# SerCharles/CN-RMA

Hardware: AMD Instinct MI355X
Metric: scenes/sec fwd (40-view->192^3 voxel): dense unprojection + RMA + voxelise + FCAF3D + decode (higher is better)
Workload: dtype f32 (sparse conv f16x3: 22-bit operands, fp32 accumulate; value_f32_conv = exact fp32); 1 GPU; NS: 40 views x 256 ch x 480x640 fp32 maps (channels_last) -> grid 192x192x192, N=300, max_points=500000, FCAF3D MinkResNet34 + head, 1 HIP graph per scene, 3 in flight; M_rows=72216505, M_selected=500000, M_unique=496819

## Files before the change

### cn-rma_amd/csrc/sparse.hip

```cpp
#include <cstdio>
#include <type_traits>
#include "common.h"

#include <hipcub/hipcub.hpp>

namespace {

struct UniqueWs {
  int32_t* slot;
  int32_t* idx;
  uint8_t* flag;
  void* scan;
  uint64_t* key_a; uint64_t* key_b;
  int32_t* val_a; int32_t* val_b;
  void* sort_tmp; size_t sort_tmp_bytes;
  int32_t* range_err;
};

size_t sort_temp_bytes(int64_t n) {
  size_t bytes = 0;
  hipError_t e = hipcub::DeviceRadixSort::SortPairs(nullptr, bytes, (const uint64_t*)nullptr, (uint64_t*)nullptr,
                                                    (const int32_t*)nullptr, (int32_t*)nullptr, (int)n, 0, 64, nullptr);
  if (e != hipSuccess || bytes == 0) bytes = (size_t)n * 16 + (1u << 20);
  (void)hipGetLastError();
// ... 1140 lines not shown
#pragma unroll
      for (int j = 0; j < 4; ++j) {
        float x = v[j];
        if (p.scale) x = x * scv[j];
        if (p.shift) x = x + shv[j];
        if (p.residual) x = x + rsv[j];
        v[j] = apply_act(x, p.act);
        mx = fmaxf(mx, fabsf(v[j]));
        if (p.out_split) store_split(p.out_split, t / p.Cout, p.Cout, col + j, v[j]);
      }
      *reinterpret_cast<float4*>(p.out + t) = make_float4(v[0], v[1], v[2], v[3]);
    } else {
      for (int j = 0; j < 4 && t + j < total; ++j) {
        float x = 0.0f;
        for (int z = 0; z < p.splits; ++z) x += p.slab[(int64_t)z * slab_stride + t + j];
        const int col = (int)((t + j) % p.Cout);
        if (p.scale) x = x * p.scale[col];
        if (p.shift) x = x + p.shift[col];
        if (p.residual) x = x + p.residual[t + j];
        x = apply_act(x, p.act);
        mx = fmaxf(mx, fabsf(x));
        p.out[t + j] = x;
      }
    }
  }
  if (p.out_amax != nullptr) {
    __shared__ float sh4[4];
    block_amax_publish(p.out_amax, mx, sh4);
  }
}

int choose_splits(int64_t rows, int Cout, int K, int bm, int bn, size_t ws_bytes) {
  if (K <= 1) return 1;
  const int64_t tiles = ceil_div(rows, bm) * ceil_div(Cout, bn);
  if (tiles >= 384) return 1;
  int s = (int)ceil_div(768, tiles);
  if (s > K) s = K;
  const size_t per = (size_t)rows * Cout * sizeof(float);
  if (per == 0) return 1;
  const int64_t fit = (int64_t)(ws_bytes / per);
  if (s > fit) s = (int)fit;
  return s < 2 ? 1 : s;
}

#ifdef CNRMA_EXPERIMENTS
#include "sparse_exp_ws.inc"
#endif

constexpr int CONV_XCD_ORDER = 0;
#ifdef CNRMA_EXPERIMENTS
constexpr int CONV_WS_SLOTS = 0;
#endif

struct ConvTune { int shape = -1; int splits = -1; int pf = -1; int ablate = 0; int ws = -1; int xcd = -1; int go = -1; int nb = -1; };
#ifdef CNRMA_EXPERIMENTS
static ConvTune g_conv_tune;
#define CNRMA_CONV_TUNE g_conv_tune
#else
static constexpr ConvTune k_conv_tune{};
#define CNRMA_CONV_TUNE k_conv_tune
#endif

enum ConvMode { CONV_EXACT = 0, CONV_F16X3 = 1, CONV_BF16 = 2 };

static int64_t capped_blocks(int64_t threads, int64_t cap) {
  const int64_t b = ceil_div(threads, 256);
  return b > cap ? cap : b;
}

static ConvArgs conv_args(const float* in, int Cin, const int32_t* nbr, int K, int Cout, float* out, int64_t no_cap,
                          const int32_t* no_dev, void* slab = nullptr) {
  ConvArgs p;
  p.in = in; p.Cin = Cin; p.nbr = nbr; p.K = K; p.Cout = Cout; p.out = out; p.no_cap = no_cap; p.no_dev = no_dev;
  p.slices = 1; p.splits = 1; p.k_per_split = K; p.slab = reinterpret_cast<float*>(slab);
  return p;
}

static ConvArgs& with_epilogue(ConvArgs& p, const float* scale, const float* shift, const float* residual, int act) {
  p.scale = scale; p.shift = shift; p.residual = residual; p.act = act;
  return p;
}

static void reduce_splits(const ConvArgs& p, hipStream_t st) {
  if (p.splits > 1)
    hipLaunchKernelGGL(conv_reduce_kernel, dim3((unsigned)capped_blocks(p.no_cap * p.Cout / 4 + 1, 4096)), dim3(256), 0, st, p);
}

enum ConvShape { T128x128, T128x64, T64x64, T128x32, T64x128, T256x128, T256x64, N_CONV_SHAPES };
struct ConvPlan { int shape, bm, bn, splits, k_per_split, pf; };

ConvPlan plan_conv(int64_t no_cap, int Cin, int Cout, int K, ConvMode mode, bool six, int slices, bool has_ws, size_t ws_bytes) {
  static const int bms[] = {128, 128, 64, 128, 64, 256, 256}, bns[] = {128, 64, 64, 32, 128, 128, 64};
  int sh;
  if (Cout <= 32) sh = T128x32;
  else if (six && mode != CONV_EXACT) {
    if (Cout >= 128) sh = no_cap >= 16384 && no_cap < 40000 ? T128x128 : (no_cap < 1000 && Cout < 256 ? T64x64 : T64x128);
    else sh = no_cap >= 200000 && Cin > 32 ? T128x64 : T64x64;
  }
  else if (six && no_cap < 1000 && Cout >= 256) sh = T64x128;
  else if (no_cap < 4000) sh = T64x64;
  else if (no_cap < 16384) sh = six ? T128x64 : T64x64;
  else if (Cout >= 128) sh = T128x128;
  else if (six && Cin <= 32) sh = T64x64;
  else sh = T128x64;
  const ConvTune t = CNRMA_CONV_TUNE;
  if (t.shape >= 0 && t.shape < N_CONV_SHAPES && (six || t.shape < T64x128) && (t.shape < T256x128 || (six && mode == CONV_F16X3 && t.ws >= 2)))
    sh = t.shape;
// ... 79 lines not shown
#ifdef CNRMA_EXPERIMENTS
    const int ws_slots = mode == CONV_F16X3 && !in_split && shape != T128x32 ? (CNRMA_CONV_TUNE.ws >= 0 ? CNRMA_CONV_TUNE.ws : CONV_WS_SLOTS) : 0;
    if (ws_slots >= 2 && CNRMA_CONV_TUNE.ablate == 0) {
      const int rc = launch_conv_ws(shape, ws_slots, has_res, grid, p, wt, st);
      if (rc != 0) return rc;
    } else
#endif
    switch (shape) {
      case T128x128: CNRMA_CONV6_LAUNCH(2, 2, 2, 2); break;
      case T128x64: CNRMA_CONV6_LAUNCH(4, 1, 1, 2); break;
      case T64x64: CNRMA_CONV6_LAUNCH(2, 2, 1, 1); break;
      case T128x32: CNRMA_CONV6_LAUNCH(4, 1, 1, 1); break;
      case T64x128: CNRMA_CONV6_LAUNCH(2, 2, 1, 2); break;
      default: return CNRMA_EINVAL;
    }
#undef CNRMA_CONV6_LAUNCH
#undef CNRMA_CONV6_ABL
    reduce_splits(p, st);
    CNRMA_LAUNCH_CHECK();
    return 0;
  }
#define CNRMA_CONV_LAUNCH(WM, WN, TM_, TN_)                                                                        \
  do {                                                                                                             \
    if (fast && has_res)                                                                                           \
      hipLaunchKernelGGL((sparse_conv_mfma_kernel<WM, WN, TM_, TN_, true, true>), grid, dim3(256), 0, st, p);      \
    else if (fast)                                                                                                 \
      hipLaunchKernelGGL((sparse_conv_mfma_kernel<WM, WN, TM_, TN_, true, false>), grid, dim3(256), 0, st, p);     \
    else if (has_res)                                                                                              \
      hipLaunchKernelGGL((sparse_conv_mfma_kernel<WM, WN, TM_, TN_, false, true>), grid, dim3(256), 0, st, p);     \
    else                                                                                                           \
      hipLaunchKernelGGL((sparse_conv_mfma_kernel<WM, WN, TM_, TN_, false, false>), grid, dim3(256), 0, st, p);    \
  } while (0)
  switch (shape) {
    case T128x128: CNRMA_CONV_LAUNCH(2, 2, 2, 2); break;
    case T128x64: CNRMA_CONV_LAUNCH(4, 1, 1, 2); break;
    case T64x64: CNRMA_CONV_LAUNCH(2, 2, 1, 1); break;
    case T128x32: CNRMA_CONV_LAUNCH(4, 1, 1, 1); break;
    default: return CNRMA_EINVAL;
  }
#undef CNRMA_CONV_LAUNCH
  reduce_splits(p, st);
  CNRMA_LAUNCH_CHECK();
  return 0;
}

constexpr int GO_BM = 64;
constexpr int GO_UMAX = 280;
constexpr int GO_HASH = 2048;
constexpr int GO_HDR = 84;
constexpr int GO_ROWS = 27 * GO_BM;

constexpr int GO_HASH_BITS = 11;
static_assert(GO_HASH == 1 << GO_HASH_BITS, "hash size");
__global__ __launch_bounds__(256) void tile_union_kernel(const int32_t* __restrict__ nbr, int64_t no_cap,
                                                         const int32_t* __restrict__ no_dev, int K,
                                                         int32_t* __restrict__ hdr, int32_t* __restrict__ rows,
                                                         uint16_t* __restrict__ lidx, int ablate) {
  __shared__ int32_t hkey[4][GO_HASH + 1];
  __shared__ __attribute__((aligned(16))) int32_t nloc[4][GO_BM * 27];
  const int wave = threadIdx.x >> 6, lane = threadIdx.x & 63;
  const int64_t tile = (int64_t)blockIdx.x * 4 + wave;
  const int64_t n_live = live_rows(no_cap, no_dev);
  const int64_t tile0 = tile * GO_BM;
  if (tile0 >= n_live) return;
  const int rows_here = (int)min((int64_t)GO_BM, n_live - tile0);
  int32_t* hk = hkey[wave];
  int32_t* nl = nloc[wave];
  uint16_t* stage = reinterpret_cast<uint16_t*>(nl);
  int32_t* th = hdr + tile * GO_HDR;
  int32_t* tr = rows + tile * GO_ROWS;
  int32_t v[27];
  {
    const int32_t* nb = nbr + tile0 * 27;
    const int total = rows_here * 27;
    int32_t f[27];
#pragma unroll
    for (int q = 0; q < 27; ++q) f[q] = q * 64 + lane < total ? nb[q * 64 + lane] : -1;
#pragma unroll
    for (int q = 0; q < 27; ++q) nl[q * 64 + lane] = f[q];
    __builtin_amdgcn_wave_barrier();
#pragma unroll
    for (int q = 0; q < 27; ++q) v[q] = nl[lane * 27 + q];
    __builtin_amdgcn_wave_barrier();
  }
  int li[27];
#pragma unroll
  for (int q = 0; q < 27; ++q) li[q] = GO_UMAX;
  unsigned valid_k = 0;
#pragma unroll
  for (int q = 0; q < 27; ++q)
    if (__ballot(v[q] >= 0) != 0ull) valid_k |= 1u << q;

  int n_groups = 0, u_begin = 0;
  unsigned cuts = 1u << 26;
  int lo = 0;
  while (lo < 27) {
    const int hi = __builtin_ctz(cuts >> lo) + lo + 1;
    const unsigned rmask = ((hi >= 32 ? 0u : (1u << hi)) - 1u) & ~((1u << lo) - 1u) & valid_k;
    if (rmask == 0u) { lo = hi; continue; }
    for (int i = lane; i < GO_HASH; i += 64) hk[i] = -1;
    __builtin_amdgcn_wave_barrier();
    int sl[27];
    unsigned pend = 0;
#pragma unroll
    for (int q = 0; q < 27; ++q) {
      sl[q] = (int)((unsigned)v[q] * 2654435761u >> (32 - GO_HASH_BITS));
      pend |= (((rmask >> q) & 1u) & (v[q] >= 0 ? 1u : 0u)) << q;
    }
    if (ablate & 32) pend = 0;
    const int max_rounds = hi - lo > GO_UMAX / GO_BM ? 8 : GO_HASH;
// ... 35 lines not shown
        const bool mine = ((act >> q) & 1u) != 0u && v[q] >= 0;
        atomicMin(&hk[mine ? sl[q] : GO_HASH], q * 64 + lane);
      }
      __builtin_amdgcn_wave_barrier();
#pragma unroll
      for (int q = 0; q < 27; ++q) {
        const bool mine = ((act >> q) & 1u) != 0u && v[q] >= 0;
        const bool owner = mine && hk[sl[q]] == q * 64 + lane;
        const unsigned long long bal = __ballot(owner);
        mypos[q] = cnt + (int)__builtin_amdgcn_mbcnt_hi((unsigned)(bal >> 32), __builtin_amdgcn_mbcnt_lo((unsigned)bal, 0u));
        own |= (owner ? 1u : 0u) << q;
        cnt += __popcll(bal);
      }
    }
    if (crowded || cnt > GO_UMAX) {
      const int len = hi - lo;
      constexpr int SURE = GO_UMAX / GO_BM;
      if (!crowded && cnt <= 2 * GO_UMAX - GO_UMAX / 4 && len > 2 * SURE) {
        cuts |= 1u << (lo + len / 2 - 1);
      } else {
        for (int c = lo + SURE; c < hi; c += SURE) cuts |= 1u << (c - 1);
      }
      continue;
    }
    const int un = cnt;
    __builtin_amdgcn_wave_barrier();
#pragma unroll
    for (int q = 0; q < 27; ++q) {
      const bool owner = ((own >> q) & 1u) != 0u;
      hk[owner ? sl[q] : GO_HASH] = mypos[q];
      if (owner) tr[u_begin + mypos[q]] = v[q];
    }
    __builtin_amdgcn_wave_barrier();
#pragma unroll
    for (int q = 0; q < 27; ++q) {
      const int r = hk[sl[q]];
      li[q] = (((rmask >> q) & 1u) != 0u && v[q] >= 0) ? r : li[q];
    }
    if (lane == 0) { th[1 + 3 * n_groups] = (int)rmask; th[2 + 3 * n_groups] = u_begin; th[3 + 3 * n_groups] = un; }
    u_begin += un;
    ++n_groups;
    lo = hi;
    __builtin_amdgcn_wave_barrier();
  }
  __builtin_amdgcn_wave_barrier();
#pragma unroll
  for (int q = 0; q < 27; ++q) stage[lane * 27 + q] = (uint16_t)li[q];
  __builtin_amdgcn_wave_barrier();
  const uint32_t* s32 = reinterpret_cast<const uint32_t*>(stage);
  uint32_t* t32 = reinterpret_cast<uint32_t*>(lidx + tile * (GO_BM * 27));
  for (int i = lane; i < GO_BM * 27 / 2; i += 64) t32[i] = s32[i];
  if (lane == 0) th[0] = n_groups;
}

struct GoArgs {
  const int32_t* hdr; const int32_t* rows; const uint16_t* lidx;
  int slices_per_split;
  unsigned* counters;
};

#ifdef CNRMA_EXPERIMENTS
#include "sparse_exp_go1.inc"
#endif

struct Go2Map { int tiles, ncol, ng, mode, per; };
__device__ __forceinline__ void go_stamp(unsigned long long* dbg, int slot) {
  unsigned long long t;
  __builtin_amdgcn_sched_barrier(0);
  asm volatile("s_memtime %0\n\ts_waitcnt lgkmcnt(0)" : "=s"(t) :: "memory");
  __builtin_amdgcn_sched_barrier(0);
  if (threadIdx.x == 0 && slot < 16) dbg[(size_t)blockIdx.x * 16 + slot] = t;
}

template <int N>
__device__ __forceinline__ void go_waitn(u32x4_t (&b)[2][2]) {
  asm volatile("s_waitcnt vmcnt(%4)" : "+v"(b[0][0]), "+v"(b[0][1]), "+v"(b[1][0]), "+v"(b[1][1]) : "n"(N));
}
__device__ __forceinline__ void go_drain(u32x4_t (&b)[2][2]) {
  asm volatile("s_waitcnt vmcnt(0)" : "+v"(b[0][0]), "+v"(b[0][1]), "+v"(b[1][0]), "+v"(b[1][1]));
}
__device__ __forceinline__ void go_load_frag(u32x4_t (&b)[2][2], const uint16_t* sbase, unsigned voff) {
  asm volatile("s_nop 4\n\t"
               "global_load_dwordx4 %0, %4, %5 offset:0\n\t"
               "global_load_dwordx4 %1, %4, %5 offset:1024\n\t"
               "global_load_dwordx4 %2, %4, %5 offset:2048\n\t"
               "global_load_dwordx4 %3, %4, %5 offset:3072"
               : "=&v"(b[0][0]), "=&v"(b[0][1]), "=&v"(b[1][0]), "=&v"(b[1][1]) : "v"(voff), "s"(sbase));
}

__device__ __forceinline__ unsigned pack_bf16x2(float lo, float hi) {
  const __bf16 a = (__bf16)lo, b = (__bf16)hi;
  return (unsigned)__builtin_bit_cast(unsigned short, a) | ((unsigned)__builtin_bit_cast(unsigned short, b) << 16);
}

template <int N>
__device__ __forceinline__ void go_waitn1(u32x4_t (&b)[2][2]) {
  asm volatile("s_waitcnt vmcnt(%2)" : "+v"(b[0][0]), "+v"(b[0][1]) : "n"(N));
}
__device__ __forceinline__ void go_drain1(u32x4_t (&b)[2][2]) {
  asm volatile("s_waitcnt vmcnt(0)" : "+v"(b[0][0]), "+v"(b[0][1]));
}
__device__ __forceinline__ void go_load_frag1(u32x4_t (&b)[2][2], const uint16_t* sbase, unsigned voff) {
  asm volatile("s_nop 4\n\t"
               "global_load_dwordx4 %0, %2, %3 offset:0\n\t"
               "global_load_dwordx4 %1, %2, %3 offset:1024"
               : "=&v"(b[0][0]), "=&v"(b[0][1]) : "v"(voff), "s"(sbase));
// ... 1667 lines not shown

__global__ __launch_bounds__(256) void kernel_map_children_kernel(const int32_t* __restrict__ parent_nbr, int64_t np_cap,
                                                                  const int32_t* __restrict__ np_dev,
                                                                  int32_t* __restrict__ nbr) {
  const int64_t n = live_rows(np_cap, np_dev) * 8;
  const int64_t e = (int64_t)blockIdx.x * blockDim.x + threadIdx.x;
  if (e >= n * 27) return;
  const int64_t t = e / 27;
  const int k = (int)(e - t * 27);
  const int64_t p = t >> 3;
  const int m = (int)(t & 7);
  const int sx = ((m >> 2) & 1) + k % 3 - 1, sy = ((m >> 1) & 1) + (k / 3) % 3 - 1, sz = (m & 1) + k / 9 - 1;
  const int px = (sx + 2) / 2 - 1, py = (sy + 2) / 2 - 1, pz = (sz + 2) / 2 - 1;
  const int kp = (pz + 1) * 9 + (py + 1) * 3 + (px + 1);
  const int mc = ((sx & 1) << 2) | ((sy & 1) << 1) | (sz & 1);
  const int32_t j = parent_nbr[p * 27 + kp];
  nbr[e] = j >= 0 ? 8 * j + mc : -1;
}

extern "C" int cnrma_sparse_kernel_map_children(const int32_t* parent_nbr, int64_t np_cap, const int32_t* np_dev, int32_t* nbr,
                                                void* stream) {
  if (parent_nbr == nullptr || nbr == nullptr || np_cap <= 0 || np_cap * 8 * 27 >= ((int64_t)1 << 40)) return CNRMA_EINVAL;
  hipLaunchKernelGGL(kernel_map_children_kernel, dim3((unsigned)ceil_div(np_cap * 8 * 27, 256)), dim3(256), 0, as_stream(stream),
                     parent_nbr, np_cap, np_dev, nbr);
  CNRMA_LAUNCH_CHECK();
  return 0;
}

extern "C" int cnrma_sparse_kernel_map_strided(const int32_t* in_coords, int64_t n_cap, const int32_t* n_dev,
                                               int in_stride, int kernel_size, const uint64_t* out_hash_keys,
                                               const int32_t* out_hash_vals, int64_t hash_cap, int32_t* nbr,
                                               int64_t no_cap, int precleared, void* stream) {
  if (n_cap <= 0 || no_cap <= 0 || in_stride <= 0 || kernel_size < 1 || kernel_size > 3) return CNRMA_EINVAL;
  const int K = kernel_size * kernel_size * kernel_size;
  hipStream_t st = as_stream(stream);
  if (!precleared) {
    hipError_t e = cnrma_fill_bytes(nbr, 0xFF, (size_t)no_cap * K * sizeof(int32_t), st);
    if (e != hipSuccess) return -(int)e;
  }
  hipLaunchKernelGGL(kernel_map_strided_kernel, dim3((unsigned)ceil_div(n_cap, 256)), dim3(256), 0, st, in_coords,
                     n_cap, n_dev, in_stride, kernel_size, out_hash_keys, out_hash_vals, hash_cap, nbr);
  CNRMA_LAUNCH_CHECK();
  return 0;
}

extern "C" size_t cnrma_sparse_conv_workspace_bytes(int64_t no_cap, int Cout, int K) {
  if (K <= 1 || no_cap >= 65536) return 0;
  return (size_t)K * (size_t)no_cap * (size_t)Cout * sizeof(float);
}

#ifdef CNRMA_EXPERIMENTS
extern "C" int cnrma_debug_conv_tuning(const int* v, int n) {
  ConvTune t;
  int* f[] = {&t.shape, &t.splits, &t.pf, &t.ablate, &t.ws, &t.xcd, &t.go, &t.nb};
  if (n < 0 || n > 8 || (n > 0 && v == nullptr)) return CNRMA_EINVAL;
  for (int i = 0; i < n; ++i) *f[i] = v[i];
  g_conv_tune = t;
  return 0;
}
#endif

extern "C" int cnrma_sparse_conv_plan(int64_t no_cap, int Cin, int Cout, int K, int mode, int slices, size_t workspace_bytes,
                                      int* out6) {
  if (out6 == nullptr || Cin <= 0 || Cout <= 0 || K <= 0 || K > 27 || no_cap <= 0 || mode < 0 || mode > 3) return CNRMA_EINVAL;
  const bool six = mode != 0 && Cin % 32 == 0;
  const ConvMode m = mode == 3 ? CONV_EXACT : static_cast<ConvMode>(mode);
  const ConvPlan pl = plan_conv(no_cap, Cin, Cout, K, m, six, slices > 1 ? slices : 1, workspace_bytes > 0, workspace_bytes);
  out6[0] = pl.bm; out6[1] = pl.bn; out6[2] = pl.splits; out6[3] = pl.k_per_split; out6[4] = pl.pf; out6[5] = pl.shape;
  return 0;
}

extern "C" int cnrma_sparse_conv_f32(const float* in_feats, int Cin, const int32_t* nbr, int K, const float* weight,
                                     int Cout, const float* scale, const float* shift, const float* residual, int act,
                                     float* out_feats, int64_t no_cap, const int32_t* no_dev, void* workspace,
                                     size_t workspace_bytes, void* stream) {
  ConvArgs p = conv_args(in_feats, Cin, nbr, K, Cout, out_feats, no_cap, no_dev, workspace);
  p.weight = weight;
  return launch_conv(with_epilogue(p, scale, shift, residual, act), CONV_EXACT, nullptr, workspace_bytes, as_stream(stream));
}

extern "C" int cnrma_sparse_conv_bf16x6(const float* in_feats, const void* in_split, int64_t in_zero_row, int Cin,
                                        const int32_t* nbr, int K, const void* weight_split, int Cout,
                                        const float* scale, const float* shift, const float* residual, int act,
                                        float* out_feats, void* out_split, int64_t no_cap, const int32_t* no_dev,
                                        void* workspace, size_t workspace_bytes, void* stream) {
  if (weight_split == nullptr || Cin % 32 != 0 || (in_feats == nullptr && in_split == nullptr)) return CNRMA_EINVAL;
  ConvArgs p = conv_args(in_feats, Cin, nbr, K, Cout, out_feats, no_cap, no_dev, workspace);
  p.in_split = reinterpret_cast<const uint16_t*>(in_split); p.in_zero_row = in_zero_row;
  p.out_split = reinterpret_cast<uint16_t*>(out_split); p.out_zero_row = no_cap;
  return launch_conv(with_epilogue(p, scale, shift, residual, act), CONV_EXACT, weight_split, workspace_bytes, as_stream(stream));
}

extern "C" int cnrma_rma_emit_features_f32(const float* feat_nhwc, const float* const* feat_nhwc_ref, int C, const void* records,
                                           int64_t n_cap, const int32_t* n_dev, const float* w_div, float* out_feat,
                                           int feat_stride, float* out_amax, void* stream) {
  if ((feat_nhwc == nullptr && feat_nhwc_ref == nullptr) || records == nullptr || out_feat == nullptr || C <= 0 || n_cap <= 0 ||
      feat_stride < C)
    return CNRMA_EINVAL;
  hipStream_t st = as_stream(stream);
  const int4* rec = reinterpret_cast<const int4*>(records);
  if (C % 256 == 0)
    hipLaunchKernelGGL((emit_features_kernel<64>), dim3((unsigned)ceil_div(n_cap * 64, 256)), dim3(256), 0, st, feat_nhwc,
                       feat_nhwc_ref, C, rec, n_cap, n_dev, w_div, out_feat, feat_stride, out_amax);
  else if (C % 32 == 0)
    hipLaunchKernelGGL((emit_features_kernel<8>), dim3((unsigned)ceil_div(n_cap * 8, 256)), dim3(256), 0, st, feat_nhwc,
                       feat_nhwc_ref, C, rec, n_cap, n_dev, w_div, out_feat, feat_stride, out_amax);
  else
    hipLaunchKernelGGL((emit_features_kernel<2>), dim3((unsigned)ceil_div(n_cap * 2, 256)), dim3(256), 0, st, feat_nhwc,
// ... 591 lines not shown

struct TileUnion { int32_t* hdr; int32_t* rows; uint16_t* lidx; size_t bytes; };
static TileUnion tile_union_view(const void* buf, int64_t no_cap) {
  const size_t tiles = (size_t)ceil_div(no_cap, GO_BM);
  const size_t hdr = align256(tiles * GO_HDR * 4), rows = align256(tiles * GO_ROWS * 4), lidx = align256(tiles * GO_BM * 27 * 2);
  const uintptr_t b = reinterpret_cast<uintptr_t>(buf);
  return {reinterpret_cast<int32_t*>(b), reinterpret_cast<int32_t*>(b + hdr), reinterpret_cast<uint16_t*>(b + hdr + rows),
          hdr + rows + lidx};
}

static GoArgs go_args(const void* tile_union, int64_t no_cap) {
  const TileUnion tu = tile_union_view(tile_union, no_cap);
  GoArgs g;
  g.hdr = tu.hdr; g.rows = tu.rows; g.lidx = tu.lidx; g.slices_per_split = 0; g.counters = nullptr;
  return g;
}

extern "C" int cnrma_sparse_conv_go_f32(const float* in_feats, int Cin, const void* tile_union, const void* weight_frag, int Cout,
                                        const float* scale, const float* shift, const float* residual, int act, float* out_feats,
                                        int64_t no_cap, const int32_t* no_dev, void* workspace, size_t workspace_bytes, void* stream) {
  if (in_feats == nullptr || tile_union == nullptr || weight_frag == nullptr || out_feats == nullptr || Cin <= 0 || Cin % BK != 0 ||
      Cout < 64 || no_cap <= 0)
    return CNRMA_EINVAL;
  hipStream_t st = as_stream(stream);
  GoArgs g = go_args(tile_union, no_cap);
  ConvArgs p = conv_args(in_feats, Cin, nullptr, 27, Cout, out_feats, no_cap, no_dev, workspace);
  with_epilogue(p, scale, shift, residual, act);
  const Go2Plan pl = go2_plan(no_cap, Cin, Cout, workspace != nullptr, workspace_bytes);
  g.slices_per_split = pl.slices_per_split;
  p.splits = pl.splits;
  const bool has_res = residual != nullptr && pl.splits == 1;
  const float* wf = reinterpret_cast<const float*>(weight_frag);
  if (pl.bn == 128) {
    if (has_res) hipLaunchKernelGGL((sparse_conv_gof_kernel<4, 1, true>), dim3(pl.blocks), dim3(256), GOF_LDS, st, p, g, wf, pl.mp);
    else hipLaunchKernelGGL((sparse_conv_gof_kernel<4, 1, false>), dim3(pl.blocks), dim3(256), GOF_LDS, st, p, g, wf, pl.mp);
  } else {
    if (has_res) hipLaunchKernelGGL((sparse_conv_gof_kernel<2, 2, true>), dim3(pl.blocks), dim3(256), GOF_LDS, st, p, g, wf, pl.mp);
    else hipLaunchKernelGGL((sparse_conv_gof_kernel<2, 2, false>), dim3(pl.blocks), dim3(256), GOF_LDS, st, p, g, wf, pl.mp);
  }
  reduce_splits(p, st);
  CNRMA_LAUNCH_CHECK();
  return 0;
}


extern "C" size_t cnrma_sparse_tile_union_bytes(int64_t no_cap) {
  return no_cap <= 0 ? 0 : tile_union_view(nullptr, no_cap).bytes;
}

extern "C" int cnrma_sparse_tile_union_build(const int32_t* nbr, int64_t no_cap, const int32_t* no_dev, int K, void* tile_union,
                                             void* stream) {
  if (nbr == nullptr || tile_union == nullptr || no_cap <= 0 || K != 27) return CNRMA_EINVAL;
  const TileUnion tu = tile_union_view(tile_union, no_cap);
  hipLaunchKernelGGL(tile_union_kernel, dim3((unsigned)ceil_div(ceil_div(no_cap, GO_BM), 4)), dim3(256), 0, as_stream(stream), nbr,
                     no_cap, no_dev, K, tu.hdr, tu.rows, tu.lidx, CNRMA_CONV_TUNE.ablate);
  CNRMA_LAUNCH_CHECK();
  return 0;
}

extern "C" int cnrma_sparse_conv_wgrad_go_bf16(const float* in_feats, int Cin, const void* tile_union, const float* grad_out,
                                               int Cout, int64_t no_cap, const int32_t* no_dev, int parts, float* slabs,
                                               void* stream) {
  if (in_feats == nullptr || tile_union == nullptr || grad_out == nullptr || slabs == nullptr || Cin <= 0 || Cout <= 0 ||
      (Cin & 3) || (Cout & 3) || no_cap <= 0 || parts <= 0)
    return CNRMA_EINVAL;
  const int64_t tiles = ceil_div(no_cap, GO_BM);
  const TileUnion tu = tile_union_view(tile_union, no_cap);
  WgoMap map;
  map.parts = parts;
  map.tiles_per_part = (int)ceil_div(tiles, parts);
  map.n_ci = (int)ceil_div(Cin, 64);
  map.n_co = (int)ceil_div(Cout, 64);
  map.by_part = parts >= 16;
  map.ablate = CNRMA_CONV_TUNE.ablate;
  const int64_t per = (int64_t)WGO_KG * map.n_ci * map.n_co;
  const int64_t blocks = (map.by_part ? ceil_div(parts, 8) * 8 : (int64_t)parts) * per;
  if (blocks > 0x7fffffffLL) return CNRMA_EINVAL;
  hipLaunchKernelGGL(conv_wgrad_go_kernel, dim3((unsigned)blocks), dim3(64 * (WGO_CW + WGO_PW)), 0, as_stream(stream), in_feats, Cin, grad_out, Cout,
                     no_cap, no_dev, tu.hdr, tu.rows, tu.lidx, slabs, map);
  CNRMA_LAUNCH_CHECK();
  return 0;
}

extern "C" int cnrma_sparse_conv_go_bf16(const float* in_feats, int Cin, const void* tile_union, const void* weight_frag, int Cout,
                                         float* out_feats, int64_t no_cap, const int32_t* no_dev, void* workspace,
                                         size_t workspace_bytes, void* stream) {
  if (in_feats == nullptr || tile_union == nullptr || weight_frag == nullptr || out_feats == nullptr || Cin <= 0 || Cin % BK != 0 ||
      Cout < 64 || no_cap <= 0)
    return CNRMA_EINVAL;
  const ConvArgs p = conv_args(in_feats, Cin, nullptr, 27, Cout, out_feats, no_cap, no_dev, workspace);
  const Go2Plan pl = go2_plan(no_cap, Cin, Cout, workspace != nullptr, workspace_bytes);
  return launch_go2(pl, p, go_args(tile_union, no_cap), reinterpret_cast<const uint16_t*>(weight_frag), false, nullptr, as_stream(stream), true);
}

extern "C" int cnrma_sparse_conv_go_f16x3(const float* in_feats, const float* in_amax, int Cin, const void* tile_union,
                                          const void* weight_frag, int Cout, const float* scale, const float* shift,
                                          const float* residual, int act, float* out_feats, float* out_amax, int64_t no_cap,
                                          const int32_t* no_dev, void* workspace, size_t workspace_bytes,
                                          void* tile_counters, void* stream) {
  if (in_feats == nullptr || in_amax == nullptr || tile_union == nullptr || weight_frag == nullptr || out_feats == nullptr ||
      Cin <= 0 || Cin % BK != 0 || Cout < 64 || no_cap <= 0)
    return CNRMA_EINVAL;
  const int K = 27;
  hipStream_t st = as_stream(stream);
  const GoArgs g = go_args(tile_union, no_cap);
  ConvArgs p = conv_args(in_feats, Cin, nullptr, K, Cout, out_feats, no_cap, no_dev, workspace);
  with_epilogue(p, scale, shift, residual, act);
  p.in_amax = in_amax; p.out_amax = out_amax;
// ... 249 lines not shown
```

### cn-rma_amd/sparse.py

```python
import ctypes
import itertools

import os
import threading

import torch
from torch.utils.weak import WeakIdKeyDictionary

from . import _lib
from . import plan as P
from ._lib import call, ptr, stream


def _next_pow2(n):
    p = 2
    while p < n:
        p *= 2
    return p


def kernel_offsets(kernel_size, tensor_stride):
    k = kernel_size
    rng = [(i - k // 2) if k % 2 == 1 else i for i in range(k)]
    offs = [(ix * tensor_stride, iy * tensor_stride, iz * tensor_stride)
# ... 524 lines not shown
    fwd, tr = hit[1:] if hit is not None else (None, None)
    if (tr if transposed else fwd) is not None:
        return _pinned(tr if transposed else fwd)
    w = weight.detach().contiguous().float()
    K, Cin, Cout = w.shape
    lib = _lib.load()
    if Cin % 32 == 0 and Cout % 32 == 0 and Cin >= 64 and fwd is None and tr is None:
        fwd = torch.empty(lib.cnrma_sparse_conv_bf16_frag_weight_bytes(K, Cin, Cout), dtype=torch.uint8, device=w.device)
        tr = torch.empty(lib.cnrma_sparse_conv_bf16_frag_weight_bytes(K, Cout, Cin), dtype=torch.uint8, device=w.device)
        call("cnrma_sparse_conv_prepare_weights_bf16_frag_pair", ptr(w), K, Cin, Cout, 1, ptr(fwd), ptr(tr), stream())
    elif transposed:
        tr = torch.empty(lib.cnrma_sparse_conv_bf16_frag_weight_bytes(K, Cout, Cin), dtype=torch.uint8, device=w.device)
        call("cnrma_sparse_conv_prepare_weights_bf16_frag", ptr(w), K, Cin, Cout, 1, 1, ptr(tr), stream())
    else:
        fwd = torch.empty(lib.cnrma_sparse_conv_bf16_frag_weight_bytes(K, Cin, Cout), dtype=torch.uint8, device=w.device)
        call("cnrma_sparse_conv_prepare_weights_bf16_frag", ptr(w), K, Cin, Cout, 0, 0, ptr(fwd), stream())
    _cache_put(weight, "_cnrma_bf16_frag", (tag, fwd, tr))
    return _pinned(tr if transposed else fwd)


def _precision(precision=None):
    if precision:
        return precision
    if torch.is_autocast_enabled() and torch.get_autocast_dtype("cuda") == torch.bfloat16:
        return "bf16"
    return CONV_PRECISION


_STAGE_IMAGE = {"bf16": weights_bf16, "f16x3": split_weights_f16, "bf16x6": split_weights}
CONV_MODES = {"f32": 0, "f16x3": 1, "bf16": 2, "bf16x6": 3}
CONV_SHAPES = ("128x128", "128x64", "64x64", "128x32", "64x128", "256x128", "256x64")


def conv_plan(n_out, Cin, Cout, K, precision=None, slices=1):
    import ctypes
    prec = precision or CONV_PRECISION
    mode = CONV_MODES[prec] if Cin % 32 == 0 else 0
    ws = _lib.load().cnrma_sparse_conv_workspace_bytes(n_out, Cout, K) if slices == 1 else 0
    out = (ctypes.c_int * 6)()
    call("cnrma_sparse_conv_plan", int(n_out), int(Cin), int(Cout), int(K), mode, int(slices), ws, out)
    return dict(tile=(out[0], out[1]), splits=out[2], k_per_split=out[3], prefetch=out[4], shape=CONV_SHAPES[out[5]])


def conv_go_plan(n_out, Cin, Cout, residual=False):
    import ctypes
    ws = _go_ws_bytes(n_out, Cin, Cout)
    out = (ctypes.c_int * 8)()
    call("cnrma_sparse_conv_go_plan", int(n_out), int(Cin), int(Cout), ws, int(bool(residual)), out)
    return dict(form=out[0], columns=out[1], ks=2 if out[1] == 64 else 1, splits=out[2], slices_per_split=out[3],
                order=("plain", "groups->xcd", "tiles->xcd")[out[4]], residual_in_kernel=bool(out[5]), blocks=out[6],
                offsets_in_flight=out[7], workspace=ws)


def conv_tuning(shape=None, splits=-1, pf=-1, ablate=0, ws=-1, xcd=-1, go=-1, nb=-1):
    import ctypes
    if shape is None and splits < 0 and pf < 0 and not ablate and ws < 0 and xcd < 0 and go < 0 and nb < 0:
        if _lib.experiments_active():
            call("cnrma_debug_conv_tuning", None, 0)
            _lib.experiments(False, "conv")
        return
    _lib.experiments(True, "conv")
    arr = (ctypes.c_int * 8)(CONV_SHAPES.index(shape) if shape is not None else -1, int(splits), int(pf), int(ablate), int(ws),
                             int(xcd), int(go), int(nb))
    call("cnrma_debug_conv_tuning", arr, 8)


GO_CONV = "auto"
GO_UMAX = 280
GO_WS_ROWS = 65536
GO_F32 = True
GO_STAMPS = None
GO_MIN_ROWS = 256
PAIR_HDR_BYTES, PAIR_OVERFLOW_WORD = 512, 64 + 34
PAIR_CONV = True
PAIR_CONV_MIN_CIN = 128


def _gather_once(in_cs, out_cs):
    if GO_CONV == "auto":
        if not in_cs.compact:
            return False
        p = P.current()
        if p is not None and p.static:
            f = p.next_flag()
            return out_cs.n >= GO_MIN_ROWS if f is None else bool(f)
        f = out_cs.n >= GO_MIN_ROWS
        if p is not None:
            p.record_flag(f)
        return f
    return bool(GO_CONV)


def _nearly_empty_map(in_cs, out_cs):
    p = P.current()
    if p is not None and p.static:
        return bool(p.next_flag())
    f = 3.375 * in_cs.n < 0.2 * 27 * out_cs.n
    if p is not None:
        p.record_flag(f)
    return f


def conv(x, weight, kernel_size=3, stride=1, scale=None, shift=None, residual=None, act=None, precision=None):
    _lib.require_gpu()
    w = weight.contiguous().float()
    if w.dim() == 2:
        w = w.unsqueeze(0)
    K, Cin, Cout = w.shape
    assert K == kernel_size ** 3 and Cin == x.F.shape[1]
    in_cs = x.cs
    out_cs = in_cs if stride == 1 else in_cs.strided(stride)
    if kernel_size == 1 and stride == 1:
        nbr = None
    else:
        nbr = in_cs.neighbours(out_cs, kernel_size, in_cs.stride)
    out = torch.empty((out_cs.n, Cout), dtype=torch.float32, device=x.device)
    out_split = out_amax = None
# ... 898 lines not shown
```

Before: 64.30 scenes/s.

## Rewrite tile-union kernel as one wave per block with shared hash/staging LDS

The tile-union build kernel now launches one 64-thread wave per tile instead of four waves per 256-thread block. It reuses the hash table's LDS for both the neighbour transpose and the 16-bit index staging, which cuts per-block shared memory so more blocks fit per CU. Per-lane index results are now written straight into LDS staging rather than held in 27 registers, and the probe loop uses byte-offset slot addressing with a dump slot to avoid branching. The old kernel is kept as a reference path selectable only in experiment builds.

```diff
diff --git a/cn-rma_amd/csrc/sparse.hip b/cn-rma_amd/csrc/sparse.hip
--- a/cn-rma_amd/csrc/sparse.hip
+++ b/cn-rma_amd/csrc/sparse.hip
@@ -1216,7 +1216,7 @@
 constexpr int CONV_WS_SLOTS = 0;
 #endif
 
-struct ConvTune { int shape = -1; int splits = -1; int pf = -1; int ablate = 0; int ws = -1; int xcd = -1; int go = -1; int nb = -1; };
+struct ConvTune { int shape = -1; int splits = -1; int pf = -1; int ablate = 0; int ws = -1; int xcd = -1; int go = -1; int nb = -1; int tu = -1; };
 #ifdef CNRMA_EXPERIMENTS
 static ConvTune g_conv_tune;
 #define CNRMA_CONV_TUNE g_conv_tune
@@ -1402,10 +1402,156 @@
 
 constexpr int GO_HASH_BITS = 11;
 static_assert(GO_HASH == 1 << GO_HASH_BITS, "hash size");
-__global__ __launch_bounds__(256) void tile_union_kernel(const int32_t* __restrict__ nbr, int64_t no_cap,
-                                                         const int32_t* __restrict__ no_dev, int K,
-                                                         int32_t* __restrict__ hdr, int32_t* __restrict__ rows,
-                                                         uint16_t* __restrict__ lidx, int ablate) {
+__global__ __launch_bounds__(64, 4) void tile_union_kernel(const int32_t* __restrict__ nbr, int64_t no_cap,
+                                                           const int32_t* __restrict__ no_dev, int K,
+                                                           int32_t* __restrict__ hdr, int32_t* __restrict__ rows,
+                                                           uint16_t* __restrict__ lidx, int ablate) {
+  __shared__ __attribute__((aligned(16))) int32_t hk[GO_HASH + 1 + GO_BM * 27 / 2];
+  static_assert(GO_BM * 27 <= GO_HASH, "the table slice fits the set");
+  int32_t* const nl = hk;
+  const int lane = threadIdx.x;
+  const int64_t tile = blockIdx.x;
+  const int64_t n_live = live_rows(no_cap, no_dev);
+  const int64_t tile0 = tile * GO_BM;
+  if (tile0 >= n_live) return;
+  const int rows_here = (int)min((int64_t)GO_BM, n_live - tile0);
+  uint16_t* stage = reinterpret_cast<uint16_t*>(hk + GO_HASH + 1);
+  int32_t* th = hdr + tile * GO_HDR;
+  int32_t* tr = rows + tile * GO_ROWS;
+  int32_t v[27];
+  {
+    const int32_t* nb = nbr + tile0 * 27;
+    const int total = rows_here * 27;
+    int32_t f[27];
+#pragma unroll
+    for (int q = 0; q < 27; ++q) f[q] = q * 64 + lane < total ? nb[q * 64 + lane] : -1;
+#pragma unroll
+    for (int q = 0; q < 27; ++q) nl[q * 64 + lane] = f[q];
+    __builtin_amdgcn_wave_barrier();
+#pragma unroll
+    for (int q = 0; q < 27; ++q) v[q] = nl[lane * 27 + q];
+    __builtin_amdgcn_wave_barrier();
+  }
+  uint16_t* const myli = stage + lane * 27;
+#pragma unroll
+  for (int q = 0; q < 27; ++q) myli[q] = (uint16_t)GO_UMAX;
+  unsigned valid_k = 0;
+#pragma unroll
+  for (int q = 0; q < 27; ++q)
+    if (__ballot(v[q] >= 0) != 0ull) valid_k |= 1u << q;
+
+  int n_groups = 0, u_begin = 0;
+  unsigned cuts = 1u << 26;
+  int lo = 0;
+  constexpr unsigned SLOT = (GO_HASH - 1) * 4, DUMP = GO_HASH * 4;
+  auto HK = [&](unsigned byte) -> int32_t& { return *reinterpret_cast<int32_t*>(reinterpret_cast<char*>(hk) + byte); };
+  while (lo < 27) {
+    const int hi = __builtin_ctz(cuts >> lo) + lo + 1;
+    const unsigned rmask = ((hi >= 32 ? 0u : (1u << hi)) - 1u) & ~((1u << lo) - 1u) & valid_k;
+    if (rmask == 0u) { lo = hi; continue; }
+    for (int i = lane; i < GO_HASH; i += 64) hk[i] = -1;
+    __builtin_amdgcn_wave_barrier();
+#pragma unroll
+    for (int q = 0; q < 27; ++q) asm volatile("" : "+v"(v[q]));
+    unsigned sl[27];
+    unsigned pend = 0;
+#pragma unroll
+    for (int q = 0; q < 27; ++q) {
+      sl[q] = ((unsigned)v[q] * 2654435761u >> (32 - GO_HASH_BITS)) << 2;
+      pend |= (((rmask >> q) & 1u) & (v[q] >= 0 ? 1u : 0u)) << q;
+    }
+    if (ablate & 32) pend = 0;
+    const int max_rounds = hi - lo > GO_UMAX / GO_BM ? 8 : GO_HASH;
+    int rounds = 0;
+    bool more = __ballot(pend != 0u) != 0ull;
+    while (more) {
+      unsigned wr = 0;
+#pragma unroll
+      for (int q = 0; q < 27; ++q) wr |= (HK(sl[q]) == -1 ? 1u : 0u) << q;
+      wr &= pend;
+      __builtin_amdgcn_wave_barrier();
+#pragma unroll
+      for (int q = 0; q < 27; ++q) HK(((wr >> q) & 1u) != 0u ? sl[q] : DUMP) = v[q];
+      __builtin_amdgcn_wave_barrier();
+      unsigned ok = 0;
+#pragma unroll
+      for (int q = 0; q < 27; ++q) ok |= (HK(sl[q]) == v[q] ? 1u : 0u) << q;
+      __builtin_amdgcn_wave_barrier();
+      pend &= ~ok;
+#pragma unroll
+      for (int q = 0; q < 27; ++q) sl[q] = (sl[q] + ((pend >> q) & 1u) * 4u) & SLOT;
+      ++rounds;
+      more = (__ballot(pend != 0u) != 0ull) & (rounds < max_rounds);
+    }
+    const bool crowded = __ballot(pend != 0u) != 0ull;
+    __builtin_amdgcn_wave_barrier();
+    const unsigned act = crowded || (ablate & 64) ? 0u : rmask;
+    unsigned mine = 0, own = 0;
+    int cnt = 0;
+#pragma unroll
+    for (int q = 0; q < 27; ++q) mine |= (((act >> q) & 1u) & (v[q] >= 0 ? 1u : 0u)) << q;
+#pragma unroll
+    for (int q = 0; q < 27; ++q) HK(((mine >> q) & 1u) != 0u ? sl[q] : DUMP) = 0x7fffffff;
+    __builtin_amdgcn_wave_barrier();
+    int ln = lane;
+    asm volatile("" : "+v"(ln));
+#pragma unroll
+    for (int q = 0; q < 27; ++q) atomicMin(&HK(((mine >> q) & 1u) != 0u ? sl[q] : DUMP), q * 64 + ln);
+    __builtin_amdgcn_wave_barrier();
+    asm volatile("" : "+v"(ln));
+#pragma unroll
+    for (int q = 0; q < 27; ++q) {
+      const bool owner = ((mine >> q) & 1u) != 0u && HK(sl[q]) == q * 64 + ln;
+      own |= (owner ? 1u : 0u) << q;
+      cnt += __popcll(__ballot(owner));
+    }
+    if (crowded || cnt > GO_UMAX) {
+      const int len = hi - lo;
+      constexpr int SURE = GO_UMAX / GO_BM;
+      if (!crowded && cnt <= 2 * GO_UMAX - GO_UMAX / 4 && len > 2 * SURE) {
+        cuts |= 1u << (lo + len / 2 - 1);
+      } else {
+        for (int c = lo + SURE; c < hi; c += SURE) cuts |= 1u << (c - 1);
+      }
+      continue;
+    }
+    const int un = cnt;
+    __builtin_amdgcn_wave_barrier();
+    int first = u_begin;
+#pragma unroll
+    for (int q = 0; q < 27; ++q) {
+      const bool owner = ((own >> q) & 1u) != 0u;
+      const unsigned long long bal = __ballot(owner);
+      const int at = first + (int)__builtin_amdgcn_mbcnt_hi((unsigned)(bal >> 32), __builtin_amdgcn_mbcnt_lo((unsigned)bal, 0u));
+      HK(owner ? sl[q] : DUMP) = at - u_begin;
+      if (owner) tr[at] = v[q];
+      first += __popcll(bal);
+    }
+    __builtin_amdgcn_wave_barrier();
+#pragma unroll
+    for (int q = 0; q < 27; ++q) {
+      if (((rmask >> q) & 1u) == 0u) continue;
+      const int r = HK(sl[q]);
+      if (v[q] >= 0) myli[q] = (uint16_t)r;
+    }
+    if (lane == 0) { th[1 + 3 * n_groups] = (int)rmask; th[2 + 3 * n_groups] = u_begin; th[3 + 3 * n_groups] = un; }
+    u_begin += un;
+    ++n_groups;
+    lo = hi;
+    __builtin_amdgcn_wave_barrier();
+  }
+  __builtin_amdgcn_wave_barrier();
+  const uint32_t* s32 = reinterpret_cast<const uint32_t*>(stage);
+  uint32_t* t32 = reinterpret_cast<uint32_t*>(lidx + tile * (GO_BM * 27));
+  for (int i = lane; i < GO_BM * 27 / 2; i += 64) t32[i] = s32[i];
+  if (lane == 0) th[0] = n_groups;
+}
+
+#ifdef CNRMA_EXPERIMENTS
+__global__ __launch_bounds__(256) void tile_union_ref_kernel(const int32_t* __restrict__ nbr, int64_t no_cap,
+                                                             const int32_t* __restrict__ no_dev, int K,
+                                                             int32_t* __restrict__ hdr, int32_t* __restrict__ rows,
+                                                             uint16_t* __restrict__ lidx, int ablate) {
   __shared__ int32_t hkey[4][GO_HASH + 1];
   __shared__ __attribute__((aligned(16))) int32_t nloc[4][GO_BM * 27];
   const int wave = threadIdx.x >> 6, lane = threadIdx.x & 63;
@@ -1547,6 +1693,7 @@
   for (int i = lane; i < GO_BM * 27 / 2; i += 64) t32[i] = s32[i];
   if (lane == 0) th[0] = n_groups;
 }
+#endif
 
 struct GoArgs {
   const int32_t* hdr; const int32_t* rows; const uint16_t* lidx;
@@ -3320,8 +3467,8 @@
 #ifdef CNRMA_EXPERIMENTS
 extern "C" int cnrma_debug_conv_tuning(const int* v, int n) {
   ConvTune t;
-  int* f[] = {&t.shape, &t.splits, &t.pf, &t.ablate, &t.ws, &t.xcd, &t.go, &t.nb};
-  if (n < 0 || n > 8 || (n > 0 && v == nullptr)) return CNRMA_EINVAL;
+  int* f[] = {&t.shape, &t.splits, &t.pf, &t.ablate, &t.ws, &t.xcd, &t.go, &t.nb, &t.tu};
+  if (n < 0 || n > 9 || (n > 0 && v == nullptr)) return CNRMA_EINVAL;
   for (int i = 0; i < n; ++i) *f[i] = v[i];
   g_conv_tune = t;
   return 0;
@@ -4019,8 +4166,16 @@
                                              void* stream) {
   if (nbr == nullptr || tile_union == nullptr || no_cap <= 0 || K != 27) return CNRMA_EINVAL;
   const TileUnion tu = tile_union_view(tile_union, no_cap);
-  hipLaunchKernelGGL(tile_union_kernel, dim3((unsigned)ceil_div(ceil_div(no_cap, GO_BM), 4)), dim3(256), 0, as_stream(stream), nbr,
-                     no_cap, no_dev, K, tu.hdr, tu.rows, tu.lidx, CNRMA_CONV_TUNE.ablate);
+#ifdef CNRMA_EXPERIMENTS
+  if (CNRMA_CONV_TUNE.tu == 0) {
+    hipLaunchKernelGGL(tile_union_ref_kernel, dim3((unsigned)ceil_div(ceil_div(no_cap, GO_BM), 4)), dim3(256), 0, as_stream(stream),
+                       nbr, no_cap, no_dev, K, tu.hdr, tu.rows, tu.lidx, CNRMA_CONV_TUNE.ablate);
+    CNRMA_LAUNCH_CHECK();
+    return 0;
+  }
+#endif
+  hipLaunchKernelGGL(tile_union_kernel, dim3((unsigned)ceil_div(no_cap, GO_BM)), dim3(GO_BM), 0, as_stream(stream), nbr, no_cap,
+                     no_dev, K, tu.hdr, tu.rows, tu.lidx, CNRMA_CONV_TUNE.ablate);
   CNRMA_LAUNCH_CHECK();
   return 0;
 }
diff --git a/cn-rma_amd/sparse.py b/cn-rma_amd/sparse.py
--- a/cn-rma_amd/sparse.py
+++ b/cn-rma_amd/sparse.py
@@ -600,17 +600,17 @@
                 offsets_in_flight=out[7], workspace=ws)
 
 
-def conv_tuning(shape=None, splits=-1, pf=-1, ablate=0, ws=-1, xcd=-1, go=-1, nb=-1):
+def conv_tuning(shape=None, splits=-1, pf=-1, ablate=0, ws=-1, xcd=-1, go=-1, nb=-1, tu=-1):
     import ctypes
-    if shape is None and splits < 0 and pf < 0 and not ablate and ws < 0 and xcd < 0 and go < 0 and nb < 0:
+    if shape is None and splits < 0 and pf < 0 and not ablate and ws < 0 and xcd < 0 and go < 0 and nb < 0 and tu < 0:
         if _lib.experiments_active():
             call("cnrma_debug_conv_tuning", None, 0)
             _lib.experiments(False, "conv")
         return
     _lib.experiments(True, "conv")
-    arr = (ctypes.c_int * 8)(CONV_SHAPES.index(shape) if shape is not None else -1, int(splits), int(pf), int(ablate), int(ws),
-                             int(xcd), int(go), int(nb))
-    call("cnrma_debug_conv_tuning", arr, 8)
+    arr = (ctypes.c_int * 9)(CONV_SHAPES.index(shape) if shape is not None else -1, int(splits), int(pf), int(ablate), int(ws),
+                             int(xcd), int(go), int(nb), int(tu))
+    call("cnrma_debug_conv_tuning", arr, 9)
 
 
 GO_CONV = "auto"
```

After: 62.90 scenes/s. 0.978x the previous value.
